# homopolymer/RAMBL

Hardware: AMD Instinct MI355X
Metric: reads/sec into POA (150bp, ~1.5k-node graph) (higher is better)
Workload: dtype f64

## Files before the change

rambl_amd/csrc/sc_api.cpp:

```cpp
#include <malloc.h>

#include <cmath>

#include "sc_ctx.hpp"

using namespace sc;
struct sc_ctx { Ctx c; sc_ctx(int device, const CtxPlan& plan) : c(device, plan) {} };

extern "C" {

int sc_host_plan(int stream_count, int local_world, double cpus, int* out) {
    if (!out || stream_count < 1) return SC_ERR_ARG;
    host_plan(stream_count, local_world > 0 ? local_world : local_world_size(), cpus > 0 ? cpus : cpu_budget_host(), out);
    return SC_OK;
}

int sc_ctx_create(int device, int stream_count, sc_ctx** out) {
    if (!out) return SC_ERR_ARG;
    *out = nullptr;
    setenv("GPU_MAX_HW_QUEUES", "16", 0);
    int ndev = 0;
    if (hipGetDeviceCount(&ndev) != hipSuccess || ndev <= 0 || device < 0 || device >= ndev) return SC_ERR_NO_DEVICE;
    hipDeviceProp_t prop;
    if (hipGetDeviceProperties(&prop, device) != hipSuccess) return SC_ERR_NO_DEVICE;
// ... 168 lines not shown
    if (!h || !n_cls || !n_pool) return SC_ERR_ARG;
    auto job = find_job(h, handle);
    if (!job || job->status != 1) return SC_ERR_ARG;
    *n_cls = (int)job->thr_count.size();
    *n_pool = (long)job->thr_pool.size();
    if (!count || !first_read || !pool || !symbols || cls_cap < *n_cls || pool_cap < *n_pool) return SC_ERR_CAPACITY;
    std::memcpy(count, job->thr_count.data(), sizeof(int) * job->thr_count.size());
    std::memcpy(first_read, job->thr_first.data(), sizeof(int) * job->thr_first.size());
    std::memcpy(pool, job->thr_pool.data(), sizeof(int) * job->thr_pool.size());
    std::memset(symbols, 0, 8);
    std::memcpy(symbols, job->thr_sym.data(), std::min<size_t>(8, job->thr_sym.size()));
    return SC_OK;
}
int sc_sample_level(sc_ctx* h, int S, const double* a0, int n_reads, const double* ll, const unsigned char* has, int n_ent,
                    int e0, const int* ent_rid, const int* ent_cn, const int* ent_sym, const int* mate_off, const int* mate_idx,
                    int n_sweeps, const double* U, int n_u, unsigned* kdraw, unsigned* cnt, long* out) {
    if (!h || !a0 || !ll || !has || !ent_rid || !ent_cn || !ent_sym || !mate_off || !U || !kdraw || !cnt || !out) return SC_ERR_ARG;
    Ctx* ctx = &h->c;
    if (ctx->resident || ctx->workers.size() != 1) return SC_ERR_ARG;
    if (S < 2 || S > MAXS || n_reads < 1 || n_ent < 1 || e0 < 0 || e0 > (1 << 20) || n_sweeps < 1) return SC_ERR_ARG;
    for (int s = 0; s < S; s++) if (!(a0[s] >= 0.0) || !std::isfinite(a0[s])) return SC_ERR_ARG;
    long Q = 0;
    for (int r = 0; r < n_ent; r++) {
        if (ent_rid[r] < 0 || ent_rid[r] >= n_reads || ent_cn[r] < 1 || ent_sym[r] < 0 || ent_sym[r] >= KMAX) return SC_ERR_ARG;
        Q += ent_cn[r];
    }
    if (Q * n_sweeps > MAX_DRAWS || n_u < Q * n_sweeps) return SC_ERR_ARG;
    for (long t = 0; t < Q * n_sweeps; t++) if (!(U[t] >= 0.0 && U[t] <= 1.0)) return SC_ERR_ARG;
    if (mate_off[0] != 0) return SC_ERR_ARG;
    for (int r = 0; r < n_reads; r++) if (mate_off[r + 1] < mate_off[r]) return SC_ERR_ARG;
    const int nm = mate_off[n_reads];
    if (nm > 0 && !mate_idx) return SC_ERR_ARG;
    for (int i = 0; i < nm; i++) if (mate_idx[i] < -1 || mate_idx[i] >= n_reads) return SC_ERR_ARG;
    try {
        Worker w;
        w.init_private(ctx);
        const int E = e0 + n_ent;
        FlatGraph f;
        f.K = KMAX; f.code_N = KMAX;
        f.ent_rid.resize((size_t)E); f.ent_cn.assign((size_t)E, 1); f.ent_lab_off.resize((size_t)E); f.ent_lab_len.assign((size_t)E, 1);
        f.ent_first.assign((size_t)E, 1);
        f.labels.assign((size_t)E + 1, 0);
        std::vector<int> qoff((size_t)E, 0);
        for (int e = 0; e < E; e++) {
            const int r = e - e0;
            f.ent_rid[(size_t)e] = r >= 0 ? ent_rid[r] : n_reads - 1 - e % n_reads;
            f.ent_lab_off[(size_t)e] = e;
            f.labels[(size_t)e] = (uint8_t)(r >= 0 ? ent_sym[r] : 0);
        }
        for (int r = 0, q = 0; r < n_ent; r++) { f.ent_cn[(size_t)(e0 + r)] = ent_cn[r]; qoff[(size_t)(e0 + r)] = q; q += ent_cn[r]; }
        const hipStream_t st = w.st;
        const std::vector<int> mptr(mate_off, mate_off + n_reads + 1), midx(mate_idx, mate_idx + nm);
        JobDev jd = w.job_dev(w.passthrough, f, qoff, mptr, midx, n_reads, std::max<long>(Q, 1), n_ent);
        auto slot = [](int s) { return (s * 37 + 5) % MAXS; };
        std::vector<double> rows((size_t)jd.ll_stride * MAXS, 0.0);
        for (int s = 0; s < S; s++) std::memcpy(&rows[(size_t)slot(s) * jd.ll_stride], ll + (size_t)s * n_reads, sizeof(double) * n_reads);
        jd.ll = upload(w.passthrough, w.b_ll, rows, st);
        std::vector<uint8_t> hv(has, has + n_reads);
        hv.resize((size_t)n_reads + 8, 0);
        jd.has = upload(w.passthrough, w.b_has, hv, st);
        std::vector<double> u(U, U + Q * n_sweeps);
        u.resize((size_t)(Q * n_sweeps + 2048), 0.5);
        std::vector<float> uf(u.begin(), u.end());
        DevBuf b_u, b_uf;
        jd.U = upload(w.passthrough, b_u, u, st);
        jd.Uf = upload(w.passthrough, b_uf, uf, st);
        const JobDev* jd_dev = (const JobDev*)w.b_jobdev.ensure(sizeof(JobDev));
        HIPCHK(hipMemcpyAsync((void*)jd_dev, &jd, sizeof jd, hipMemcpyHostToDevice, st));

        LevelParams& P = *w.Ph;
        for (int s = 0; s < S; s++) P.sp[s] = StrainParam{slot(s), E, 1, 0, a0[s], 0.0};
        LevelHdr H{};
        H.mode = MODE_SAMPLE; H.S = S; H.e0 = e0; H.e1 = E; H.Q = (int)Q; H.n_sweeps = n_sweeps;
        H.n_copy = 0; H.do_update = 0; H.seq = 1;
        std::memset(w.Rh, 0, sizeof(LevelResult));
        LevelBatch batch;
// ... 45 lines not shown
```

rambl_amd/csrc/sc_ctx.hpp:

```cpp
#pragma once
#include <atomic>
#include <condition_variable>
#include <deque>
#include <map>
#include <memory>
#include <mutex>
#include <thread>

#include "../../include/straincall_hip.h"
#include "sc_device.hpp"
#include "sc_fiber.hpp"
#include "sc_graph.hpp"
#include "sc_host.hpp"
#include "sc_plan.hpp"

namespace sc {

void launch_edge_support(hipStream_t st, const int* out_ptr, const int* out_node, const int* pool_ptr, const int* pool_rid,
                         const int* pool_cn, const uint8_t* node_is_end, const int* edge_src, int n_edges, int sorted,
                         int* support);
bool level_wants_grid(const JobDev& job, const LevelHdr& h);
int launch_level_grid(hipStream_t st, const JobDev& job, const LevelHdr& h, const LevelParams* Pd, LevelResult* R);
int level_kind(const LevelHdr& h);
int level_lds_kb(const LevelHdr& h, int K);
// ... 144 lines not shown
    Fiber* fib = nullptr;
    int slot = 0;
    hipStream_t st = nullptr;
    bool own_stream = false;
    hipEvent_t sync_ev = nullptr;
    std::atomic<int> level_state{0};
    std::string level_err;
    double t_seen = 0, wake_acc[2] = {0, 0};
    std::atomic<int> mslot{-1};
    std::atomic<double> t_posted{0};
    double t_batch_launched = 0;
    int batch_n = 0;
    hipEvent_t ev0 = nullptr, ev1 = nullptr;
    std::vector<hipEvent_t> ev_pool;
    size_t ev_used = 0;
    LevelParams* Ph = nullptr;
    LevelParams* Pm = nullptr;
    LevelParams* Pd = nullptr;
    LevelResult* Rh = nullptr;
    LevelResult* Rd = nullptr;
    bool own_blocks = false;
    unsigned seq = 0;
    DevBuf b_ent_rid, b_ent_cn, b_ent_lab_off, b_ent_lab_len, b_ent_first, b_ent_qoff, b_labels, b_mate_ptr, b_mate_idx,
        b_ll, b_has, b_isnew, b_tabA, b_tabLf, b_qcode, b_qent, b_quid, b_out_ptr, b_out_node, b_pool_ptr, b_pool_rid,
        b_pool_cn, b_isend, b_esrc, b_support, b_jobdev;
    DevBuf m_seqs, m_off, m_cols0, m_cols1, m_counts, m_moves, m_trace, m_out, m_edge;
    PinnedArena* stage = nullptr;
    PinnedArena passthrough;
    DevBuf t_ref, t_pos, t_seqoff, t_seq, t_cigoff, t_cigop, t_ciglen, t_lut, t_tabs, t_pool, t_pool2;
    FlatGraph flat;
    std::vector<int> ent_qoff_buf;
    bool setup_held = false;
    std::vector<ld> cnt_scratch;

    ~Worker();
    void init();
    void init_private(Ctx* c);
    void run();
    void process(Job& job);
    void complete_level(const LevelItem& it, bool timed);
    void wait_level();
    void finish_level(int state, const char* err = nullptr);
    void sync_stream();
    int msa_device(const std::vector<std::string>& seqs, std::vector<std::string>& rows);
    void thread_device(const std::string& G, const std::vector<AlignedRead>& R, const std::vector<std::vector<CigarOp>>& cig,
                       ThreadTables& T);
    JobDev job_dev(PinnedArena& ar, const FlatGraph& f, const std::vector<int>& ent_qoff, const std::vector<int>& mate_off,
                   const std::vector<int>& mate_idx, int n_reads, long qcap, int max_entries);
    LevelItem level_item(const JobDev* job, const LevelHdr& H, int K) const {
        return LevelItem{job, H, level_kind(H) | (level_lds_kb(H, K) << 8), Pm, Rd};
    }
    void cluster(Job& job, const PoGraph& g, FlatGraph& f);
};
struct MailHold {
    Worker* w;
    void drop() { const int m = w->mslot.load(std::memory_order_relaxed); if (m >= 0) { w->mslot.store(-1, std::memory_order_release); w->grid->release_mailbox(m); } }
    ~MailHold() { drop(); }
};

void walk_levels(Worker& w, Job& job, const FlatGraph& f, const JobDev& jd, const JobDev* jd_dev, const std::vector<int>& level_hi,
                 int final_e0, long total_copies, MailHold& mail);
bool gpu_local_cpus(int device, cpu_set_t* out);

}
```

rambl_amd/csrc/sc_device.hpp:

```cpp
#pragma once
#include <cstdint>

namespace sc {

constexpr int MAXS = 128;
constexpr int KMAX = 16;
constexpr int KK = KMAX * KMAX;
constexpr int MAX_DRAWS = 40000;

enum LevelMode { MODE_HARD = 0, MODE_SAMPLE = 1 };

struct JobDev {
    const int* ent_rid;
    const int* ent_cn;
    const int* ent_lab_off;
    const int* ent_lab_len;
    const uint8_t* ent_first;
    const int* ent_qoff;
    const uint8_t* labels;
    const int* mate_ptr;
    const int* mate_idx;
    int n_reads;
    int K;
    int code_N;
    double* ll;
    long ll_stride;
    uint8_t* has;
    const double* U;
    const float* Uf;
    uint8_t* isnew;
    double* tabA;
    float* tabLf;
    uint8_t* qcode;
    int* qent;
    int* quid;
    long qcap;
};

struct LevelHdr {
    int mode;
    int S;
    int e0, e1;
    int has_dups;
    int any_multi;
    int Q;
    int n_sweeps;
    int n_copy;
    int do_update;
    int done;
    int copy_n;
    unsigned seq;
};
struct StrainParam {
    int slot;
    int lab_off, lab_len;
    int pad;
    double a0;
    double logpri;
};
// ... 93 lines not shown
```

rambl_amd/csrc/sc_kernels.hip:

```cpp
#include <hip/hip_runtime.h>
#include <math.h>
#include <stdint.h>
#include <stdlib.h>

#include "sc_device.hpp"

namespace sc {

#define SC_GLOBAL __attribute__((address_space(1)))
#define SC_LDS __attribute__((address_space(3)))

constexpr int LDS_TOTAL = 160 * 1024 - 256;
constexpr int LDS_SMALL = 18 * 1024;
constexpr int LDS_BIG = LDS_TOTAL - LDS_SMALL;
static_assert(LDS_SMALL >= (int)(sizeof(double) * 2 * MAXS + sizeof(StrainParam) * MAXS + sizeof(unsigned) * MAXS * KMAX + sizeof(int) * 6 * MAXS + 64), "LDS_SMALL");
static_assert(LDS_BIG >= (int)(sizeof(double) * MAXS * 64), "LDS_BIG");

template <int CTRL, int ROW_MASK, int BANK_MASK, bool BOUND>
__device__ __forceinline__ double dpp_f64(double v) {
    int lo = __double2loint(v), hi = __double2hiint(v);
    lo = __builtin_amdgcn_update_dpp(0, lo, CTRL, ROW_MASK, BANK_MASK, BOUND);
    hi = __builtin_amdgcn_update_dpp(0, hi, CTRL, ROW_MASK, BANK_MASK, BOUND);
    return __hiloint2double(hi, lo);
}
// ... 160 lines not shown
}
__device__ __forceinline__ f2v pk_sub(f2v a, f2v b) {
    f2v d;
    asm("v_pk_add_f32 %0, %1, %2 neg_lo:[0,1] neg_hi:[0,1]" : "=v"(d) : "v"(a), "v"(b));
    return d;
}
__device__ __forceinline__ unsigned min3_u32(unsigned m, unsigned x, unsigned y) {
    unsigned d;
    asm("v_min3_u32 %0, %1, %2, %3" : "=v"(d) : "v"(m), "v"(x), "v"(y));
    return d;
}
template <int QP> __device__ __forceinline__ float quad_f32(float v) {
    return __int_as_float(__builtin_amdgcn_update_dpp(0, __float_as_int(v), QP, 0xF, 0xF, true));
}
template <int QP> __device__ __forceinline__ int quad_i32(int v) {
    return __builtin_amdgcn_update_dpp(0, v, QP, 0xF, 0xF, true);
}
__device__ __forceinline__ void lds_barrier() { asm volatile("s_waitcnt lgkmcnt(0)\n\ts_barrier" ::: "memory"); }

constexpr int UWIN = 1024;
#ifdef SC_CHAIN_PROF
__device__ unsigned long long g_chain_prof[12];
#define CHAIN_STAMP(k) do { if (wv == 0) { const unsigned long long t_ = clock64(); prof[k] += t_ - tprev; tprev = t_; } } while (0)
#else
#define CHAIN_STAMP(k) do {} while (0)
#endif

template <int NQ, bool ROWS_LDS, int NW, class JD>
__device__ __forceinline__ void urn_chain_q(const JD& job, const LevelHdr& h, const StrainParam* s_sp, LevelResult* __restrict__ R,
                                            const int* s_slot, volatile double* s_a, volatile double* s_p, unsigned* s_kf,
                                            const float* s_a0f, unsigned* s_cnt, int* s_x, float* s_uwin, const float* rows_lds, int stride, int tid) {
    constexpr int SPL = 4 * NQ, SP = 16 * NQ;
    constexpr int NPLC = SP > 64 ? 2 : 1;
    constexpr float EPSW = (float)(SP + 16) * 1.5e-7f;
    const int lane = tid & 63, wv = __builtin_amdgcn_readfirstlane(tid >> 6), k = lane & 3, pos = wv * 16 + (lane >> 2);
    const int S = h.S, Q = h.Q, n = h.n_sweeps, e0 = h.e0;
    const int Sm1 = S - 1;
    const int total = n * Q;
    const SlowArgs sa{job.qent, job.quid, job.ent_rid, job.ll, job.ll_stride, job.has};
    const SC_GLOBAL double* Ustream = (const SC_GLOBAL double*)job.U;
    const SC_GLOBAL float* Uf = (const SC_GLOBAL float*)job.Uf;
    const SC_GLOBAL float* rows_g = (const SC_GLOBAL float*)job.tabLf;
    auto ld4 = [&](int idx) __attribute__((always_inline)) -> f4v {
        return ROWS_LDS ? *(const f4v*)(rows_lds + idx) : *(const SC_GLOBAL f4v*)(rows_g + idx);
    };
    auto ld1 = [&](int idx) __attribute__((always_inline)) -> float { return ROWS_LDS ? rows_lds[idx] : rows_g[idx]; };

    const int cbase = k * SPL;
    const float m0 = k > 0 ? 1.0f : 0.0f, m1 = k > 1 ? 1.0f : 0.0f;
    const float posf = (float)pos + 1.0e-37f;
    double a0m[NPLC];
#pragma unroll
    for (int i = 0; i < NPLC; i++) { const int s = lane * NPLC + i; a0m[i] = (s < S) ? s_sp[s].a0 : 0.0; }
    f4v a0q[NQ];
#pragma unroll
    for (int g = 0; g < NQ; g++) a0q[g] = *(const f4v*)(s_a0f + cbase + 4 * g);
    unsigned long long n_exact = 0, n_slow = 0, n_pass = 0;
    const unsigned long long clk0 = clock64(), wall0 = wall_clock64();

    int ulo = 0;
    bool upf = false;
    f4v ux0 = 0.0f, ux1 = 0.0f;
    if (wv == 0) {
#pragma unroll
        for (int j = 0; j < UWIN / 256; j++) *(f4v*)(s_uwin + 256 * j + 4 * lane) = *(const SC_GLOBAL f4v*)(Uf + 256 * j + 4 * lane);
    }
    __syncthreads();

    int t = 0;
    int ro = (pos % Q) * stride;
    const int wrap = Q * stride;
    int upos = pos;
    f4v L[NQ];
    float uf = 0.0f, llast = 0.0f;
    int sym = 0;
    auto issue_loads = [&]() __attribute__((always_inline)) {
#pragma unroll
        for (int g = 0; g < NQ; g++) L[g] = ld4(ro + cbase + 4 * g);
        llast = ld1(ro + Sm1);
        sym = __float_as_int(ld1(ro + S));
        uf = s_uwin[upos];
    };
    if (total > 0) issue_loads();
#ifdef SC_CHAIN_PROF
    unsigned long long prof[5] = {0, 0, 0, 0, 0}, tprev = clock64();
#endif
#pragma unroll 1
    while (t < total) {
        asm volatile("" ::: "memory");
        n_pass++;
        float loc[SPL];
        float run = 0.0f;
        u4v kq[NQ];
#pragma unroll
        for (int g = 0; g < NQ; g++) kq[g] = *(const u4v*)(s_kf + cbase + 4 * g);
        const unsigned klast = s_kf[Sm1];
        const float a0last = s_a0f[Sm1];
#pragma unroll
        for (int g = 0; g < NQ; g++) {
            const u4v kk = kq[g];
            const f4v av = a0q[g] + f4v{(float)kk.x, (float)kk.y, (float)kk.z, (float)kk.w};
            loc[4 * g + 0] = run = (g == 0) ? av.x * L[g].x : fma_rn(av.x, L[g].x, run);
            loc[4 * g + 1] = run = fma_rn(av.y, L[g].y, run);
            loc[4 * g + 2] = run = fma_rn(av.z, L[g].z, run);
            loc[4 * g + 3] = run = fma_rn(av.w, L[g].w, run);
        }
        const float alast = a0last + (float)klast;
        CHAIN_STAMP(0);
// ... 34 lines not shown
        int adv = 16 * NW;
#pragma unroll
        for (int j = 0; j < NW / 4; j++) {
            const i4v xf = *(const i4v*)(s_x + 4 * j);
            adv = min(adv, min(min(xf.x, xf.y), min(xf.z, xf.w)));
        }
        adv = adv < rem ? adv : rem;
        CHAIN_STAMP(2);
        if (adv == 0) {
            if (wv == 0) {
                const double u = Ustream[t];
                double ad[NPLC];
#pragma unroll
                for (int i = 0; i < NPLC; i++) { const int s = lane * NPLC + i; ad[i] = a0m[i] + (double)((s < S) ? s_kf[s] : 0u); }
                const int qi = __builtin_amdgcn_readfirstlane(ro) / stride;
                const int cc = slow_draw<NPLC>(sa, s_slot, s_a, s_p, ad[0], NPLC > 1 ? ad[NPLC - 1] : 0.0, S, qi, e0, u, lane);
                n_slow++;
                n_exact += (cc >> 8) & 1;
                c = cc & 0xFF;
            }
            adv = 1;
        }
        const bool acc = (pos < adv) && (k == 0);
        const int cs = c * KMAX + sym;
        const bool accs = acc && (sym < KMAX);
        t += adv;
        if (t >= total) {
            if (acc) __hip_atomic_fetch_add(&s_kf[c], 1u, __ATOMIC_RELAXED, __HIP_MEMORY_SCOPE_WORKGROUP);
            if (accs) __hip_atomic_fetch_add(&s_cnt[cs], 1u, __ATOMIC_RELAXED, __HIP_MEMORY_SCOPE_WORKGROUP);
            break;
        }
        if (Q >= 16 * NW) {
            const unsigned r1 = (unsigned)(ro + adv * stride);
            const unsigned r2 = r1 - (unsigned)wrap;
            ro = (int)(r1 < r2 ? r1 : r2);
        } else {
            ro = ((ro / stride + adv) % Q) * stride;
        }
        upos = (upos + adv) & (UWIN - 1);
        if (wv == 0) {
            if (!upf && t >= ulo + UWIN / 4) {
                ux0 = *(const SC_GLOBAL f4v*)(Uf + ulo + UWIN + 4 * lane);
                ux1 = *(const SC_GLOBAL f4v*)(Uf + ulo + UWIN + 256 + 4 * lane);
                upf = true;
            }
            if (t >= ulo + UWIN / 2) {
                *(f4v*)(s_uwin + ((ulo & (UWIN - 1)) + 4 * lane)) = ux0;
                *(f4v*)(s_uwin + ((ulo & (UWIN - 1)) + 256 + 4 * lane)) = ux1;
                ulo += UWIN / 2;
                upf = false;
            }
        }
        issue_loads();
        if (acc) __hip_atomic_fetch_add(&s_kf[c], 1u, __ATOMIC_RELAXED, __HIP_MEMORY_SCOPE_WORKGROUP);
        if (accs) __hip_atomic_fetch_add(&s_cnt[cs], 1u, __ATOMIC_RELAXED, __HIP_MEMORY_SCOPE_WORKGROUP);
        CHAIN_STAMP(3);
        lds_barrier();
        CHAIN_STAMP(4);
    }
#ifdef SC_CHAIN_PROF
    if (tid == 0) { for (int i = 0; i < 5; i++) atomicAdd(&g_chain_prof[i], prof[i]); atomicAdd(&g_chain_prof[5], n_pass); }
#endif
    __syncthreads();
    if (wv == 0) {
#pragma unroll
        for (int i = 0; i < NPLC; i++) {
            const int s = lane * NPLC + i;
            if (s < S) { R->abund[s] = a0m[i] + (double)s_kf[s]; R->kdraw[s] = s_kf[s]; }
        }
        if (lane == 0) {
            R->n_draws = (unsigned long long)total; R->n_exact = n_exact; R->n_slow = n_slow; R->n_pass = n_pass;
            R->chain_cycles = clock64() - clk0; R->chain_wall = wall_clock64() - wall0;
        }
    }
}

template <int NW>
__device__ __forceinline__ void urn_chain_shadow(const LevelHdr& h, const int* s_x) {
    const int total = h.n_sweeps * h.Q;
    __syncthreads();
    int t = 0;
#pragma unroll 1
    while (t < total) {
        lds_barrier();
        int adv = 16 * NW;
#pragma unroll
        for (int j = 0; j < NW / 4; j++) {
            const i4v xf = *(const volatile i4v*)(s_x + 4 * j);
            adv = min(adv, min(min(xf.x, xf.y), min(xf.z, xf.w)));
        }
        const int rem = total - t;
        adv = adv < rem ? adv : rem;
        if (adv == 0) adv = 1;
        t += adv;
        if (t >= total) break;
        lds_barrier();
// ... 364 lines not shown
    }
    phase_copies(job, h, l.s_copy, tid, nt);
    if (tid == 0) R->phase_ticks[1] = (unsigned)(wall_clock64() - wall0);
    if (upd) {
        phase_slots<false>(job, h, tid, nt);
        phase_update(job, h, l.s_sp, l.s_lab, reinterpret_cast<const double*>(l.s_big), tid, nt);
    }
    if (tid == 0) R->phase_ticks[2] = (unsigned)(wall_clock64() - wall0);
    if (!upd) phase_slots(job, h, tid, nt);
    if (tid == 0) R->phase_ticks[3] = (unsigned)(wall_clock64() - wall0);

    {
        constexpr int SR = (NB <= 2) ? 16 * NB : 16;
        const long lstride = job.ll_stride;
        SC_GLOBAL float* rows_g = (SC_GLOBAL float*)job.tabLf;
        auto put4 = [&](long idx, f4v v) __attribute__((always_inline)) {
            if (ROWS_LDS) *(f4v*)(s_rows + idx) = v; else *(SC_GLOBAL f4v*)(rows_g + idx) = v;
        };
        const float qnanf = __int_as_float(0x7fc00000);
        for (int q = tid; q < Q; q += nt) {
            const int rid = job.ent_rid[e0 + job.qent[q]], uid = job.quid[q];
            const bool hr = h.do_update ? true : job.has[rid] != 0;
            const bool hu = uid >= 0 && job.has[uid] != 0;
            const int c0 = job.qcode[q];
            const float symf = __int_as_float(c0 < KMAX ? c0 : KMAX);
            const long Lf = (long)q * stride;
            auto cell = [&](int sx) __attribute__((always_inline)) -> double {
                const double* row = job.ll + (long)l.s_slot[sx] * lstride;
                double v = hr ? row[rid] : 0.0;
                if (hu) v += row[uid];
                return v;
            };
            double m = -INFINITY;
            double x[SR];
            if (NB <= 2) {
#pragma unroll
                for (int i = 0; i < SR; i++) { x[i] = -INFINITY; if (i < S) { x[i] = cell(i); m = fmax(m, x[i]); } }
            } else {
                for (int s0 = 0; s0 < S; s0 += SR) {
#pragma unroll
                    for (int i = 0; i < SR; i++) if (s0 + i < S) m = fmax(m, cell(s0 + i));
                }
            }
            const bool flag = !(m >= -600.0);
            for (int s0 = 0; s0 < stride; s0 += SR) {
                if (NB > 2) {
#pragma unroll
                    for (int i = 0; i < SR; i++) x[i] = (s0 + i < S) ? cell(s0 + i) : -INFINITY;
                }
#pragma unroll
                for (int i = 0; i < SR; i += 4) {
                    if (s0 + i < stride) {
                        f4v w;
#pragma unroll
                        for (int k = 0; k < 4; k++) {
                            const int sx = s0 + i + k;
                            const float wk = sx < S ? (flag ? qnanf : exp_weight(x[i + k] - m)) : (sx == S ? symf : 0.0f);
                            if (k == 0) w.x = wk; else if (k == 1) w.y = wk; else if (k == 2) w.z = wk; else w.w = wk;
                        }
                        put4(Lf + s0 + i, w);
                    }
                }
            }
            if (q == Q - 1) for (int i = 0; i < 16; i += 4) put4(Lf + stride + i, f4v{0.0f, 0.0f, 0.0f, 0.0f});
        }
    }
    __syncthreads();
    if (tid == 0) R->phase_ticks[4] = (unsigned)(wall_clock64() - wall0);
    constexpr int NW = chain_nw(NB);
    if (tid >= 64 * NW) {
        if (!STAY) return;
        urn_chain_shadow<NW>(h, l.s_x);
    } else {
        urn_chain_q<NB, ROWS_LDS, NW>(job, h, l.s_sp, R, l.s_slot, l.s_a, l.s_p, l.s_kf, l.s_a0f, l.s_cnt, l.s_x, s_uwin, s_rows, stride, tid);
    }
    if (!STAY) nt = 64 * NW;
    __syncthreads();
    for (int i = tid; i < S * KMAX; i += nt) R->cnt[i] = l.s_cnt[i];
    finish_level(h, R, wall0, tid);
}

template <class IT>
__device__ __forceinline__ void level_plain_body(const IT& it, unsigned char* s_raw) {
    const unsigned long long wall0 = wall_clock64();
    const LevelHdr h = load_hdr(it);
    KJob& job = *(KJob*)it.job;
    const LevelParams* __restrict__ P = it.P;
    LevelResult* __restrict__ R = it.R;
    const LevelLds l = level_lds(s_raw);
    double* s_tab = reinterpret_cast<double*>(l.s_big);
    const int tid = threadIdx.x, nt = blockDim.x;
    const int S = h.S, K = job.K, K2 = K * K, e0 = h.e0, Rn = h.e1 - h.e0;
    const long stride = job.ll_stride;
    const bool upd = h.do_update && Rn > 0;
    stage_params(h, P, l.s_sp, l.s_copy, s_tab, upd && !(h.done & LV_ITEMS_DONE), K2, tid, nt);
    if (tid == 0) { R->error = 0; R->n_draws = 0; R->n_exact = 0; R->n_slow = 0; R->n_pass = 0; R->chain_cycles = 0; R->chain_wall = 0; }
    __syncthreads();
    if (tid == 0) R->phase_ticks[0] = (unsigned)(wall_clock64() - wall0);
    if (tid < S) l.s_lab[tid] = (int)job.labels[l.s_sp[tid].lab_off];
// ... 686 lines not shown
```

rambl_amd/csrc/sc_region.cpp:

```cpp
#include "sc_ctx.hpp"

namespace sc {

int Worker::msa_device(const std::vector<std::string>& seqs, std::vector<std::string>& rows) {
    const int n = (int)seqs.size();
    std::vector<int> off(n + 1, 0);
    std::string packed;
    for (int i = 0; i < n; i++) { packed += seqs[i]; off[i + 1] = (int)packed.size(); }
    const int cmax = (int)packed.size() + 1;
    size_t longest = 0;
    for (int i = 1; i < n; i++) longest = std::max(longest, seqs[i].size());
    MsaDev d;
    char* dseq = (char*)m_seqs.ensure(packed.size() + 1);
    int* doff = (int*)m_off.ensure(sizeof(int) * (n + 1));
    stage->h2d(dseq, packed.data(), packed.size(), st);
    stage->h2d(doff, off.data(), sizeof(int) * (n + 1), st);
    d.seqs = dseq; d.seq_off = doff; d.n = n; d.cmax = cmax;
    d.cols[0] = (char*)m_cols0.ensure((size_t)cmax * n);
    d.cols[1] = (char*)m_cols1.ensure((size_t)cmax * n);
    d.counts = (int*)m_counts.ensure(sizeof(int) * 11 * (size_t)cmax);
    d.mv_stride = (int)((longest + 1 + 63) / 64) * 64;
    d.moves = (uint8_t*)m_moves.ensure((size_t)(cmax + 1) * (size_t)d.mv_stride);
    d.edge = (int*)m_edge.ensure(sizeof(int) * 2 * (size_t)(cmax + 1));
    d.trace = (int*)m_trace.ensure(sizeof(int) * 2 * (size_t)(cmax + 64));
// ... 90 lines not shown
    T.tmin.resize((size_t)ncls * 8); T.off.resize((size_t)ncls + 1); T.pool.resize((size_t)m_bases);
    int err = 0;
    stage->d2h(T.count.data(), d.count, sizeof(int) * (size_t)ncls, st);
    stage->d2h(T.minrid.data(), d.minrid, sizeof(int) * (size_t)ncls, st);
    stage->d2h(T.smin.data(), d.smin, sizeof(int) * (size_t)ncls, st);
    stage->d2h(T.emin.data(), d.emin, sizeof(int) * (size_t)ncls, st);
    stage->d2h(T.tmin.data(), d.tmin, sizeof(int) * (size_t)ncls * 8, st);
    stage->d2h(T.off.data(), d.off, sizeof(int) * ((size_t)ncls + 1), st);
    stage->d2h(T.pool.data(), pool_sorted, sizeof(int) * (size_t)std::max<long>(m_bases, 0), st);
    stage->d2h(&err, d.err, sizeof(int), st);
    const double t_sync0 = now_ms();
    sync_stream();
    stage->land();
    if (ctx->plan.opt.sync_log) fprintf(stderr, "sync thread_device %.3f ms\n", now_ms() - t_sync0);
    SC_DPHASE("downloads");
#undef SC_DPHASE
    if (err) throw ScError(SC_ERR_ARG, "a read runs outside the window or past its own bases");
    const int INF = 0x7fffffff;
    auto fix = [&](std::vector<int>& v) { for (int& x : v) if (x == 0x7f7f7f7f) x = INF; };
    fix(T.minrid); fix(T.smin); fix(T.emin); fix(T.tmin);
}

JobDev Worker::job_dev(PinnedArena& ar, const FlatGraph& f, const std::vector<int>& ent_qoff, const std::vector<int>& mate_off,
                       const std::vector<int>& mate_idx, int n_reads, long qcap, int max_entries) {
    JobDev jd{};
    jd.ent_rid = upload(ar, b_ent_rid, f.ent_rid, st);
    jd.ent_cn = upload(ar, b_ent_cn, f.ent_cn, st);
    jd.ent_lab_off = upload(ar, b_ent_lab_off, f.ent_lab_off, st);
    jd.ent_lab_len = upload(ar, b_ent_lab_len, f.ent_lab_len, st);
    jd.ent_first = upload(ar, b_ent_first, f.ent_first, st);
    jd.ent_qoff = upload(ar, b_ent_qoff, ent_qoff, st);
    jd.labels = upload(ar, b_labels, f.labels, st);
    jd.mate_ptr = upload(ar, b_mate_ptr, mate_off, st);
    jd.mate_idx = upload(ar, b_mate_idx, mate_idx, st);
    jd.n_reads = n_reads; jd.K = f.K; jd.code_N = f.code_N;
    jd.ll_stride = ((long)n_reads + 3) & ~3L;
    jd.isnew = (uint8_t*)b_isnew.ensure((size_t)max_entries + 8);
    jd.qcap = qcap;
    jd.tabA = (double*)b_tabA.ensure(sizeof(double) * (size_t)qcap * MAXS);
    jd.tabLf = (float*)b_tabLf.ensure(sizeof(float) * (size_t)(std::min<long>(qcap, MAX_DRAWS) + 4) * 136);
    jd.qcode = (uint8_t*)b_qcode.ensure((size_t)qcap + 8);
    jd.qent = (int*)b_qent.ensure(sizeof(int) * (size_t)qcap);
    jd.quid = (int*)b_quid.ensure(sizeof(int) * (size_t)qcap);
    return jd;
}

void Worker::cluster(Job& job, const PoGraph& g, FlatGraph& f) {
    const int n_reads = (int)job.reads.size();
    const double t_cluster0 = now_ms();

    const int final_e0 = (int)f.ent_rid.size();
    long total_copies = 0;
    {
        int qo = 0;
        for (int i = 0; i < n_reads; i++) {
            f.ent_rid.push_back(i); f.ent_cn.push_back(job.reads[i].cn); f.ent_lab_off.push_back(0);
            f.ent_lab_len.push_back(0); f.ent_first.push_back(1);
            qo += job.reads[i].cn;
        }
        total_copies = qo;
    }
    std::vector<int>& ent_qoff = ent_qoff_buf;
    ent_qoff.assign(f.ent_rid.size(), 0);
    int max_level_entries = n_reads, max_level_q = 0;
    for (int l = 0; l < f.n_levels; l++) {
        int qo = 0;
        for (int x = f.level_ent_ptr[l]; x < f.level_ent_ptr[l + 1]; x++) { ent_qoff[x] = qo; qo += f.ent_cn[x]; }
        max_level_entries = std::max(max_level_entries, f.level_ent_ptr[l + 1] - f.level_ent_ptr[l]);
        max_level_q = std::max(max_level_q, qo);
    }
    { int qo = 0; for (int i = 0; i < n_reads; i++) { ent_qoff[final_e0 + i] = qo; qo += job.reads[i].cn; } }
    const long qcap = std::max<long>(std::max<long>(max_level_q, total_copies), 1);
    std::vector<int> level_hi((size_t)f.n_levels + 1, 0);
    for (int l = 0; l < f.n_levels; l++) {
        int hi = level_hi[(size_t)l];
        for (int x = f.level_ent_ptr[l]; x < f.level_ent_ptr[l + 1]; x++) {
            const int rid = f.ent_rid[x];
            hi = std::max(hi, rid + 1);
            for (int k = job.mate_off[(size_t)rid]; k < job.mate_off[(size_t)rid + 1]; k++) hi = std::max(hi, job.mate_idx[(size_t)k] + 1);
        }
        level_hi[(size_t)l + 1] = hi;
    }

    JobDev jd = job_dev(*stage, f, ent_qoff, job.mate_off, job.mate_idx, n_reads, qcap, max_level_entries);
    jd.ll = (double*)b_ll.ensure(sizeof(double) * (size_t)jd.ll_stride * MAXS);
    jd.has = (uint8_t*)b_has.ensure((size_t)n_reads + 8);
    HIPCHK(hipMemsetAsync(jd.has, 0, (size_t)n_reads + 8, st));
    jd.U = ctx->U.d.p;
    jd.Uf = ctx->U.f.p;
    const JobDev* jd_dev = (const JobDev*)b_jobdev.ensure(sizeof(JobDev));
    stage->h2d((void*)jd_dev, &jd, sizeof jd, st);

    {
        std::vector<int> esrc(f.out_node.size());
        for (int a = 0; a < f.n_nodes; a++) for (int x = f.out_ptr[a]; x < f.out_ptr[a + 1]; x++) esrc[x] = a;
        int* d_out_ptr = upload(*stage, b_out_ptr, f.out_ptr, st);
        int* d_out_node = upload(*stage, b_out_node, f.out_node, st);
        int* d_pool_ptr = upload(*stage, b_pool_ptr, f.pool_ptr, st);
        int* d_pool_rid = upload(*stage, b_pool_rid, f.pool_rid, st);
        int* d_pool_cn = upload(*stage, b_pool_cn, f.pool_cn, st);
        uint8_t* d_isend = upload(*stage, b_isend, f.node_is_end, st);
        int* d_esrc = upload(*stage, b_esrc, esrc, st);
        int* d_sup = (int*)b_support.ensure(sizeof(int) * std::max<size_t>(esrc.size(), 1));
        launch_edge_support(st, d_out_ptr, d_out_node, d_pool_ptr, d_pool_rid, d_pool_cn, d_isend, d_esrc, (int)esrc.size(),
                            f.pools_sorted ? 1 : 0, d_sup);
        if (!esrc.empty())
            stage->d2h(f.out_support.data(), d_sup, sizeof(int) * esrc.size(), st);
// ... 67 lines not shown
```

rambl_amd/csrc/sc_walk.cpp:

```cpp
#include <cmath>

#include "sc_ctx.hpp"

namespace sc {

struct Model {
    int ks = KMAX;
    ld sub[KK];
    ld comp[6]; ld Z;
    ld lsub[KK];
    double lpc[KK];
    uint16_t stale[KMAX];
    unsigned dirty;
    Model() = default;
    Model(const Model& o) { *this = o; }
    Model& operator=(const Model& o) {
        ks = o.ks; Z = o.Z; dirty = o.dirty;
        const size_t n = (size_t)ks * ks;
        std::memcpy(sub, o.sub, sizeof(ld) * n); std::memcpy(lsub, o.lsub, sizeof(ld) * n); std::memcpy(lpc, o.lpc, sizeof(double) * n);
        std::memcpy(comp, o.comp, sizeof comp); std::memcpy(stale, o.stale, sizeof stale);
        return *this;
    }
};
struct HStrain {
// ... 218 lines not shown
            sp.slot = sv[s].slot;
            sp.lab_off = sv[s].node >= 0 ? f.node_lab_off[sv[s].node] : 0;
            sp.lab_len = sv[s].node >= 0 ? f.node_lab_len[sv[s].node] : 0;
            la_cache[s] = (sp.lab_len == 1) ? (int)f.labels[(size_t)sp.lab_off] : -1;
            sp.pad = 0;
            sp.a0 = (double)sv[s].abundance;
            sp.logpri = (mode == MODE_HARD) ? (double)logl(sv[s].abundance / za) : 0.0;
            if (!do_update) continue;
            Model& hm = models[(size_t)sv[s].model];
            for (int a = 0; a < K; a++) {
                if (!(hm.dirty & (1u << a))) continue;
                const ld lc = logl(a < 6 ? hm.comp[a] : (ld)0);
                for (int b = 0; b < K; b++) {
                    if (hm.stale[a] & (1u << b)) hm.lsub[a * K + b] = logl(hm.sub[a * K + b]);
                    hm.lpc[a * K + b] = (double)(hm.lsub[a * K + b] - lc);
                }
                hm.stale[a] = 0;
            }
            hm.dirty = 0;
            double* dst = P.lpt + (size_t)s * K * K;
            std::memcpy(dst, hm.lpc, sizeof(double) * (size_t)K * K);
        }
        const bool chain = (mode == MODE_SAMPLE) && S > 1 && n_sweeps > 0;
        const bool timed = chain && pa.want_timing && !w.grid;
        if (level_wants_grid(jd, H)) {
            const size_t bytes = offsetof(LevelParams, lpt) + sizeof(double) * (size_t)S * K * K;
            HIPCHK(hipMemcpyAsync(w.Pd, w.Ph, bytes, hipMemcpyHostToDevice, w.st));
            H.done = launch_level_grid(w.st, jd, H, w.Pd, w.Rd);
            w.sync_stream();
        }
        const int ms = w.mslot.load(std::memory_order_relaxed);
        H.seq = ms >= 0 ? ++w.grid->mail_seq[(size_t)ms] : ++w.seq;
        if (timed) {
            if (w.ev_used + 2 > w.ev_pool.size()) {
                hipEvent_t a = nullptr, b = nullptr;
                HIPCHK(hipEventCreate(&a)); HIPCHK(hipEventCreate(&b));
                w.ev_pool.push_back(a); w.ev_pool.push_back(b);
            }
            w.ev0 = w.ev_pool[w.ev_used]; w.ev1 = w.ev_pool[w.ev_used + 1];
            w.ev_used += 2;
        }
        const double t_launched = level_log ? now_ms() : 0.0;
        lap(0);
        const LevelItem it = w.level_item(jd_dev, H, K);
        w.complete_level(it, timed);
        t_mark = now_ms();
// ... 2 lines not shown
        if (chain) {
            stats.sampler_launches++; stats.sampler_read_copies += Q;
            stats.draws += (long)Rh->n_draws; stats.exact_draws += (long)Rh->n_exact; stats.slow_draws += (long)Rh->n_slow;
            stats.sampler_strains += S; stats.chain_passes += (long)Rh->n_pass;
            stats.chain_cycles += (long)Rh->chain_cycles; stats.chain_wall_ticks += (long)Rh->chain_wall;
        }
        stats.level_kernel_ticks += (long)Rh->level_wall;
        if (chain) stats.sampler_level_ticks += (long)Rh->level_wall;
        if (level_log) {
            const double t_done = now_ms();
            fprintf(level_log, "h %d mode %d S %d Q %d n %d level_us %.1f chain_us %.1f cyc %llu passes %llu slow %llu xcc %d ncopy %d multi %d "
                    "ph %.1f %.1f %.1f %.1f %.1f host_us %.1f wait_us %.1f pend_us %.1f batch %d\n", job.handle, mode, S, Q,
                    n_sweeps, Rh->level_wall * 0.01, chain ? Rh->chain_wall * 0.01 : 0.0, chain ? (unsigned long long)Rh->chain_cycles : 0ull,
                    chain ? (unsigned long long)Rh->n_pass : 0ull, chain ? (unsigned long long)Rh->n_slow : 0ull, Rh->xcc, H.n_copy, (int)any_multi,
                    Rh->phase_ticks[0] * 0.01, Rh->phase_ticks[1] * 0.01, Rh->phase_ticks[2] * 0.01, Rh->phase_ticks[3] * 0.01, Rh->phase_ticks[4] * 0.01,
                    1e3 * (t_launched - t_last_done), 1e3 * (t_done - t_launched), 1e3 * (w.t_batch_launched - t_launched), w.batch_n);
            t_last_done = t_done;
        }
        stats.xcd_levels[Rh->xcc & 7]++;
        stats.kind_levels[std::min(std::max(it.kind & 0xFF, 0), 16)]++;
    }
    void np_bayes_clustering(int e0, int e1, int Q, bool has_dups, bool any_multi) {
        const int S = (int)level_strains.size();
        const int n = std::min(pa.sweeps_cap, pa.draw_budget / Q);
        int last[MAXS];
        for (int s = 0; s < S; s++) {
            last[s] = s;
            for (int t = S - 1; t > s; t--)
                if (level_strains[t].hash == level_strains[s].hash && level_strains[t].seqlen == level_strains[s].seqlen) { last[s] = t; break; }
        }
        ld prior[MAXS], post[MAXS], a[MAXS];
        for (int s = 0; s < S; s++) prior[s] = level_strains[last[s]].abundance;
        run_level(MODE_SAMPLE, e0, e1, Q, n, true, level_strains, has_dups, any_multi);
        ld (*cnt)[KMAX] = reinterpret_cast<ld (*)[KMAX]>(w.cnt_scratch.data());
        for (int s = 0; s < S; s++) {
            const Model& m_ = models[(size_t)level_strains[s].model];
            __builtin_prefetch(&Rh->cnt[s * KMAX]);
            if ((s & 15) == 0) __builtin_prefetch(&Rh->kdraw[s]);
            __builtin_prefetch(&m_.comp[0]); __builtin_prefetch(&m_.comp[4]); __builtin_prefetch(&m_.stale[0]);
            const int la = la_cache[s];
            if (la >= 0 && la < K) { __builtin_prefetch(&m_.sub[la * K]); __builtin_prefetch(&m_.sub[la * K + 4]); }
        }
        for (int s = 0; s < S; s++) for (int b = 0; b < K; b++) cnt[s][b] = 0;
        if (S == 1 || n <= 0) {
            a[0] = level_strains[0].abundance;
            for (int s = 1; s < S; s++) a[s] = level_strains[s].abundance;
            if (n > 0) {
// ... 120 lines not shown
            if (first_child[cands[c].parent] == c) { ns.slot = par.slot; ns.model = par.model; }
            else {
                if (free_slots.empty()) throw ScError(SC_ERR_CAPACITY, "out of read_loglik rows");
                ns.slot = free_slots.back(); free_slots.pop_back();
                pending_copies.push_back({par.slot, ns.slot});
                ns.model = model_new();
                models[(size_t)ns.model] = models[(size_t)par.model];
            }
            arena.push_back({cands[c].node, par.tail});
            ns.tail = (int)arena.size() - 1; ns.node = cands[c].node;
            ns.hash = hash_extend(par.hash, f.node_label_str[cands[c].node]);
            ns.seqlen = par.seqlen + (int)f.node_label_str[cands[c].node].size();
            ns.abundance = cands[c].abundance;
            sub_strains.push_back(ns);
        }
        level_strains.swap(sub_strains);
        sub_strains.clear();
    }
    void read_assign() {
        std::vector<HStrain>& fs = final_strains;
        const int S = (int)fs.size();
        if (S == 0) return;
        const int Q = (int)total_copies;
        const int n = std::min(pa.sweeps_cap, pa.draw_budget / std::max(Q, 1));
        std::vector<ld> a(S);
        if (S == 1 || n <= 0) {
            for (int s = 0; s < S; s++) a[s] = fs[s].abundance;
            if (n > 0) a[0] = sc_add_ones(a[0], (unsigned long)((long)n * Q));
        } else {
            pending_copies.clear();
            run_level(MODE_SAMPLE, final_e0, final_e0 + n_reads, Q, n, false, fs, false, true);
            for (int s = 0; s < S; s++) {
                a[s] = sc_add_ones(fs[s].abundance, Rh->kdraw[s]);
            }
        }
        mail.drop();
        if (w.ctx->gate.split_exec && FiberPool::in_fiber()) FiberPool::yield();
        ld z = 0;
        for (int s = 0; s < S; s++) z += a[s];
        for (int s = 0; s < S; s++) fs[s].abundance = a[s] / z;
        sort_strains(fs);
        for (auto& s : fs) {
            job.seqs.push_back(path_seq(s, true));
            job.abund.push_back((double)s.abundance);
        }
    }
    void report() {
// ... 66 lines not shown
```

Before: 14660.

## Log per-draw strain choices to a global buffer and tally symbol counts afterward

The urn chain loop no longer loads each copy's symbol and no longer does a second LDS atomic per accepted draw. Instead it writes the chosen strain byte to a global draw log. After the chain, a separate pass rebuilds the strain×symbol count table by run-length scanning the log in parallel. This shortens the serial per-draw critical path, including one fewer load and one fewer atomic per step. In exchange it adds global byte stores, a post-pass over all Q·n draws, and a sized device buffer with a capacity check on the host.

```diff
diff --git a/rambl_amd/csrc/sc_api.cpp b/rambl_amd/csrc/sc_api.cpp
--- a/rambl_amd/csrc/sc_api.cpp
+++ b/rambl_amd/csrc/sc_api.cpp
@@ -214,7 +214,8 @@
     for (int s = 0; s < S; s++) if (!(a0[s] >= 0.0) || !std::isfinite(a0[s])) return SC_ERR_ARG;
     long Q = 0;
     for (int r = 0; r < n_ent; r++) {
-        if (ent_rid[r] < 0 || ent_rid[r] >= n_reads || ent_cn[r] < 1 || ent_sym[r] < 0 || ent_sym[r] >= KMAX) return SC_ERR_ARG;
+        const bool sym_ok = (ent_sym[r] >= 0 && ent_sym[r] < KMAX) || ent_sym[r] == 0xFF;
+        if (ent_rid[r] < 0 || ent_rid[r] >= n_reads || ent_cn[r] < 1 || !sym_ok) return SC_ERR_ARG;
         Q += ent_cn[r];
     }
     if (Q * n_sweeps > MAX_DRAWS || n_u < Q * n_sweeps) return SC_ERR_ARG;
@@ -243,7 +244,7 @@
         for (int r = 0, q = 0; r < n_ent; r++) { f.ent_cn[(size_t)(e0 + r)] = ent_cn[r]; qoff[(size_t)(e0 + r)] = q; q += ent_cn[r]; }
         const hipStream_t st = w.st;
         const std::vector<int> mptr(mate_off, mate_off + n_reads + 1), midx(mate_idx, mate_idx + nm);
-        JobDev jd = w.job_dev(w.passthrough, f, qoff, mptr, midx, n_reads, std::max<long>(Q, 1), n_ent);
+        JobDev jd = w.job_dev(w.passthrough, f, qoff, mptr, midx, n_reads, std::max<long>(Q, 1), n_ent, Q * n_sweeps);
         auto slot = [](int s) { return (s * 37 + 5) % MAXS; };
         std::vector<double> rows((size_t)jd.ll_stride * MAXS, 0.0);
         for (int s = 0; s < S; s++) std::memcpy(&rows[(size_t)slot(s) * jd.ll_stride], ll + (size_t)s * n_reads, sizeof(double) * n_reads);
diff --git a/rambl_amd/csrc/sc_ctx.hpp b/rambl_amd/csrc/sc_ctx.hpp
--- a/rambl_amd/csrc/sc_ctx.hpp
+++ b/rambl_amd/csrc/sc_ctx.hpp
@@ -190,7 +190,7 @@
     bool own_blocks = false;
     unsigned seq = 0;
     DevBuf b_ent_rid, b_ent_cn, b_ent_lab_off, b_ent_lab_len, b_ent_first, b_ent_qoff, b_labels, b_mate_ptr, b_mate_idx,
-        b_ll, b_has, b_isnew, b_tabA, b_tabLf, b_qcode, b_qent, b_quid, b_out_ptr, b_out_node, b_pool_ptr, b_pool_rid,
+        b_ll, b_has, b_isnew, b_tabA, b_tabLf, b_qcode, b_qent, b_quid, b_dlog, b_out_ptr, b_out_node, b_pool_ptr, b_pool_rid,
         b_pool_cn, b_isend, b_esrc, b_support, b_jobdev;
     DevBuf m_seqs, m_off, m_cols0, m_cols1, m_counts, m_moves, m_trace, m_out, m_edge;
     PinnedArena* stage = nullptr;
@@ -214,12 +214,13 @@
     void thread_device(const std::string& G, const std::vector<AlignedRead>& R, const std::vector<std::vector<CigarOp>>& cig,
                        ThreadTables& T);
     JobDev job_dev(PinnedArena& ar, const FlatGraph& f, const std::vector<int>& ent_qoff, const std::vector<int>& mate_off,
-                   const std::vector<int>& mate_idx, int n_reads, long qcap, int max_entries);
+                   const std::vector<int>& mate_idx, int n_reads, long qcap, int max_entries, long max_draws);
     LevelItem level_item(const JobDev* job, const LevelHdr& H, int K) const {
         return LevelItem{job, H, level_kind(H) | (level_lds_kb(H, K) << 8), Pm, Rd};
     }
     void cluster(Job& job, const PoGraph& g, FlatGraph& f);
 };
+inline int level_sweeps(const sc_params& pa, long Q) { return (int)std::min<long>(pa.sweeps_cap, pa.draw_budget / std::max<long>(Q, 1)); }
 struct MailHold {
     Worker* w;
     void drop() { const int m = w->mslot.load(std::memory_order_relaxed); if (m >= 0) { w->mslot.store(-1, std::memory_order_release); w->grid->release_mailbox(m); } }
diff --git a/rambl_amd/csrc/sc_device.hpp b/rambl_amd/csrc/sc_device.hpp
--- a/rambl_amd/csrc/sc_device.hpp
+++ b/rambl_amd/csrc/sc_device.hpp
@@ -35,6 +35,8 @@
     int* qent;
     int* quid;
     long qcap;
+    uint8_t* dlog;
+    long dlog_cap;
 };
 
 struct LevelHdr {
diff --git a/rambl_amd/csrc/sc_kernels.hip b/rambl_amd/csrc/sc_kernels.hip
--- a/rambl_amd/csrc/sc_kernels.hip
+++ b/rambl_amd/csrc/sc_kernels.hip
@@ -206,14 +206,16 @@
 #ifdef SC_CHAIN_PROF
 __device__ unsigned long long g_chain_prof[12];
 #define CHAIN_STAMP(k) do { if (wv == 0) { const unsigned long long t_ = clock64(); prof[k] += t_ - tprev; tprev = t_; } } while (0)
+#define CHAIN_STAMP_W(k) do { asm volatile("s_waitcnt lgkmcnt(0)" ::: "memory"); CHAIN_STAMP(k); } while (0)
 #else
 #define CHAIN_STAMP(k) do {} while (0)
+#define CHAIN_STAMP_W(k) do {} while (0)
 #endif
 
 template <int NQ, bool ROWS_LDS, int NW, class JD>
 __device__ __forceinline__ void urn_chain_q(const JD& job, const LevelHdr& h, const StrainParam* s_sp, LevelResult* __restrict__ R,
                                             const int* s_slot, volatile double* s_a, volatile double* s_p, unsigned* s_kf,
-                                            const float* s_a0f, unsigned* s_cnt, int* s_x, float* s_uwin, const float* rows_lds, int stride, int tid) {
+                                            const float* s_a0f, int* s_x, float* s_uwin, const float* rows_lds, int stride, int tid) {
     constexpr int SPL = 4 * NQ, SP = 16 * NQ;
     constexpr int NPLC = SP > 64 ? 2 : 1;
     constexpr float EPSW = (float)(SP + 16) * 1.5e-7f;
@@ -225,6 +227,7 @@
     const SC_GLOBAL double* Ustream = (const SC_GLOBAL double*)job.U;
     const SC_GLOBAL float* Uf = (const SC_GLOBAL float*)job.Uf;
     const SC_GLOBAL float* rows_g = (const SC_GLOBAL float*)job.tabLf;
+    SC_GLOBAL unsigned char* dlog = (SC_GLOBAL unsigned char*)job.dlog;
     auto ld4 = [&](int idx) __attribute__((always_inline)) -> f4v {
         return ROWS_LDS ? *(const f4v*)(rows_lds + idx) : *(const SC_GLOBAL f4v*)(rows_g + idx);
     };
@@ -257,17 +260,15 @@
     int upos = pos;
     f4v L[NQ];
     float uf = 0.0f, llast = 0.0f;
-    int sym = 0;
     auto issue_loads = [&]() __attribute__((always_inline)) {
 #pragma unroll
         for (int g = 0; g < NQ; g++) L[g] = ld4(ro + cbase + 4 * g);
         llast = ld1(ro + Sm1);
-        sym = __float_as_int(ld1(ro + S));
         uf = s_uwin[upos];
     };
     if (total > 0) issue_loads();
 #ifdef SC_CHAIN_PROF
-    unsigned long long prof[5] = {0, 0, 0, 0, 0}, tprev = clock64();
+    unsigned long long prof[9] = {0, 0, 0, 0, 0, 0, 0, 0, 0}, tprev = clock64();
 #endif
 #pragma unroll 1
     while (t < total) {
@@ -348,12 +349,10 @@
             adv = 1;
         }
         const bool acc = (pos < adv) && (k == 0);
-        const int cs = c * KMAX + sym;
-        const bool accs = acc && (sym < KMAX);
+        SC_GLOBAL unsigned char* const lg = dlog + (t + pos);
         t += adv;
         if (t >= total) {
-            if (acc) __hip_atomic_fetch_add(&s_kf[c], 1u, __ATOMIC_RELAXED, __HIP_MEMORY_SCOPE_WORKGROUP);
-            if (accs) __hip_atomic_fetch_add(&s_cnt[cs], 1u, __ATOMIC_RELAXED, __HIP_MEMORY_SCOPE_WORKGROUP);
+            if (acc) { __hip_atomic_fetch_add(&s_kf[c], 1u, __ATOMIC_RELAXED, __HIP_MEMORY_SCOPE_WORKGROUP); *lg = (unsigned char)c; }
             break;
         }
         if (Q >= 16 * NW) {
@@ -377,16 +376,20 @@
                 upf = false;
             }
         }
+        CHAIN_STAMP(3);
         issue_loads();
+        CHAIN_STAMP_W(6);
         if (acc) __hip_atomic_fetch_add(&s_kf[c], 1u, __ATOMIC_RELAXED, __HIP_MEMORY_SCOPE_WORKGROUP);
-        if (accs) __hip_atomic_fetch_add(&s_cnt[cs], 1u, __ATOMIC_RELAXED, __HIP_MEMORY_SCOPE_WORKGROUP);
-        CHAIN_STAMP(3);
+        CHAIN_STAMP_W(7);
+        if (acc) *lg = (unsigned char)c;
+        CHAIN_STAMP_W(8);
         lds_barrier();
         CHAIN_STAMP(4);
     }
 #ifdef SC_CHAIN_PROF
-    if (tid == 0) { for (int i = 0; i < 5; i++) atomicAdd(&g_chain_prof[i], prof[i]); atomicAdd(&g_chain_prof[5], n_pass); }
+    if (tid == 0) { for (int i = 0; i < 9; i++) if (i != 5) atomicAdd(&g_chain_prof[i], prof[i]); atomicAdd(&g_chain_prof[5], n_pass); }
 #endif
+    asm volatile("s_waitcnt vmcnt(0)" ::: "memory");
     __syncthreads();
     if (wv == 0) {
 #pragma unroll
@@ -398,6 +401,41 @@
             R->n_draws = (unsigned long long)total; R->n_exact = n_exact; R->n_slow = n_slow; R->n_pass = n_pass;
             R->chain_cycles = clock64() - clk0; R->chain_wall = wall_clock64() - wall0;
         }
+    }
+}
+
+template <class JD>
+__device__ __forceinline__ void draw_log_counts(const JD& job, const LevelHdr& h, unsigned* s_cnt, int tid, int nt) {
+    const int Q = h.Q, n = h.n_sweeps;
+    if (Q <= 0 || n <= 0) return;
+    __builtin_amdgcn_fence(__ATOMIC_ACQUIRE, "agent");
+    const SC_GLOBAL unsigned char* dlog = (const SC_GLOBAL unsigned char*)job.dlog;
+    const int G = Q < nt ? min(nt / Q, n) : 1;
+    const int per = (n + G - 1) / G;
+    for (int idx = tid; idx < Q * G; idx += nt) {
+        const int q = idx % Q, j0 = (idx / Q) * per, j1 = min(j0 + per, n);
+        const int sym = job.qcode[q];
+        if (sym >= KMAX || j0 >= j1) continue;
+        const SC_GLOBAL unsigned char* p = dlog + (j0 * Q + q);
+        int cur = 0;
+        unsigned run = 0;
+        auto count = [&](int c) __attribute__((always_inline)) {
+            if (c != cur) {
+                if (run) __hip_atomic_fetch_add(&s_cnt[cur * KMAX + sym], run, __ATOMIC_RELAXED, __HIP_MEMORY_SCOPE_WORKGROUP);
+                cur = c; run = 0;
+            }
+            run++;
+        };
+        int j = j0;
+        for (; j + 8 <= j1; j += 8, p += 8 * Q) {
+            int c[8];
+#pragma unroll
+            for (int i = 0; i < 8; i++) c[i] = p[i * Q] & (MAXS - 1);
+#pragma unroll
+            for (int i = 0; i < 8; i++) count(c[i]);
+        }
+        for (; j < j1; j++, p += Q) count(*p & (MAXS - 1));
+        if (run) __hip_atomic_fetch_add(&s_cnt[cur * KMAX + sym], run, __ATOMIC_RELAXED, __HIP_MEMORY_SCOPE_WORKGROUP);
     }
 }
 
@@ -808,8 +846,6 @@
             const int rid = job.ent_rid[e0 + job.qent[q]], uid = job.quid[q];
             const bool hr = h.do_update ? true : job.has[rid] != 0;
             const bool hu = uid >= 0 && job.has[uid] != 0;
-            const int c0 = job.qcode[q];
-            const float symf = __int_as_float(c0 < KMAX ? c0 : KMAX);
             const long Lf = (long)q * stride;
             auto cell = [&](int sx) __attribute__((always_inline)) -> double {
                 const double* row = job.ll + (long)l.s_slot[sx] * lstride;
@@ -841,7 +877,7 @@
 #pragma unroll
                         for (int k = 0; k < 4; k++) {
                             const int sx = s0 + i + k;
-                            const float wk = sx < S ? (flag ? qnanf : exp_weight(x[i + k] - m)) : (sx == S ? symf : 0.0f);
+                            const float wk = sx < S ? (flag ? qnanf : exp_weight(x[i + k] - m)) : 0.0f;
                             if (k == 0) w.x = wk; else if (k == 1) w.y = wk; else if (k == 2) w.z = wk; else w.w = wk;
                         }
                         put4(Lf + s0 + i, w);
@@ -858,9 +894,10 @@
         if (!STAY) return;
         urn_chain_shadow<NW>(h, l.s_x);
     } else {
-        urn_chain_q<NB, ROWS_LDS, NW>(job, h, l.s_sp, R, l.s_slot, l.s_a, l.s_p, l.s_kf, l.s_a0f, l.s_cnt, l.s_x, s_uwin, s_rows, stride, tid);
+        urn_chain_q<NB, ROWS_LDS, NW>(job, h, l.s_sp, R, l.s_slot, l.s_a, l.s_p, l.s_kf, l.s_a0f, l.s_x, s_uwin, s_rows, stride, tid);
     }
     if (!STAY) nt = 64 * NW;
+    draw_log_counts(job, h, l.s_cnt, tid, nt);
     __syncthreads();
     for (int i = tid; i < S * KMAX; i += nt) R->cnt[i] = l.s_cnt[i];
     finish_level(h, R, wall0, tid);
diff --git a/rambl_amd/csrc/sc_region.cpp b/rambl_amd/csrc/sc_region.cpp
--- a/rambl_amd/csrc/sc_region.cpp
+++ b/rambl_amd/csrc/sc_region.cpp
@@ -136,7 +136,7 @@
 }
 
 JobDev Worker::job_dev(PinnedArena& ar, const FlatGraph& f, const std::vector<int>& ent_qoff, const std::vector<int>& mate_off,
-                       const std::vector<int>& mate_idx, int n_reads, long qcap, int max_entries) {
+                       const std::vector<int>& mate_idx, int n_reads, long qcap, int max_entries, long max_draws) {
     JobDev jd{};
     jd.ent_rid = upload(ar, b_ent_rid, f.ent_rid, st);
     jd.ent_cn = upload(ar, b_ent_cn, f.ent_cn, st);
@@ -156,6 +156,8 @@
     jd.qcode = (uint8_t*)b_qcode.ensure((size_t)qcap + 8);
     jd.qent = (int*)b_qent.ensure(sizeof(int) * (size_t)qcap);
     jd.quid = (int*)b_quid.ensure(sizeof(int) * (size_t)qcap);
+    jd.dlog_cap = std::max<long>(max_draws, 1);
+    jd.dlog = (uint8_t*)b_dlog.ensure((size_t)jd.dlog_cap + 8);
     return jd;
 }
 
@@ -185,6 +187,9 @@
     }
     { int qo = 0; for (int i = 0; i < n_reads; i++) { ent_qoff[final_e0 + i] = qo; qo += job.reads[i].cn; } }
     const long qcap = std::max<long>(std::max<long>(max_level_q, total_copies), 1);
+    auto level_draws = [&](long Q) { return (long)level_sweeps(job.params, Q) * Q; };
+    long max_draws = level_draws(total_copies);
+    for (int l = 0; l < f.n_levels; l++) max_draws = std::max(max_draws, level_draws(f.level_read_count[(size_t)l]));
     std::vector<int> level_hi((size_t)f.n_levels + 1, 0);
     for (int l = 0; l < f.n_levels; l++) {
         int hi = level_hi[(size_t)l];
@@ -196,7 +201,7 @@
         level_hi[(size_t)l + 1] = hi;
     }
 
-    JobDev jd = job_dev(*stage, f, ent_qoff, job.mate_off, job.mate_idx, n_reads, qcap, max_level_entries);
+    JobDev jd = job_dev(*stage, f, ent_qoff, job.mate_off, job.mate_idx, n_reads, qcap, max_level_entries, max_draws);
     jd.ll = (double*)b_ll.ensure(sizeof(double) * (size_t)jd.ll_stride * MAXS);
     jd.has = (uint8_t*)b_has.ensure((size_t)n_reads + 8);
     HIPCHK(hipMemsetAsync(jd.has, 0, (size_t)n_reads + 8, st));
diff --git a/rambl_amd/csrc/sc_walk.cpp b/rambl_amd/csrc/sc_walk.cpp
--- a/rambl_amd/csrc/sc_walk.cpp
+++ b/rambl_amd/csrc/sc_walk.cpp
@@ -264,6 +264,7 @@
             std::memcpy(dst, hm.lpc, sizeof(double) * (size_t)K * K);
         }
         const bool chain = (mode == MODE_SAMPLE) && S > 1 && n_sweeps > 0;
+        if (mode == MODE_SAMPLE && (long)n_sweeps * Q > jd.dlog_cap) throw ScError(SC_ERR_INTERNAL, "a level draws more than the region's draw log holds");
         const bool timed = chain && pa.want_timing && !w.grid;
         if (level_wants_grid(jd, H)) {
             const size_t bytes = offsetof(LevelParams, lpt) + sizeof(double) * (size_t)S * K * K;
@@ -312,7 +313,7 @@
     }
     void np_bayes_clustering(int e0, int e1, int Q, bool has_dups, bool any_multi) {
         const int S = (int)level_strains.size();
-        const int n = std::min(pa.sweeps_cap, pa.draw_budget / Q);
+        const int n = level_sweeps(pa, Q);
         int last[MAXS];
         for (int s = 0; s < S; s++) {
             last[s] = s;
@@ -479,7 +480,7 @@
         const int S = (int)fs.size();
         if (S == 0) return;
         const int Q = (int)total_copies;
-        const int n = std::min(pa.sweeps_cap, pa.draw_budget / std::max(Q, 1));
+        const int n = level_sweeps(pa, Q);
         std::vector<ld> a(S);
         if (S == 1 || n <= 0) {
             for (int s = 0; s < S; s++) a[s] = fs[s].abundance;
```

Result: faster. 15120 (median of 6 runs) (+3.2%).
